# junhong-3dv/s2m2

Measured on AMD Instinct MI355X. Metric: stereo pairs/sec, S-model 1216x1024 fp16 refine_iter=3 (ms/pair = 1000*n_gpus/value), higher is better.
Workload: dtype f16; 1 GPU; S-model 1216x1024 refine_iter=3 use_positivity=True, 1 pair(s) per GPU per step, random-init weights (seeded LeCun normal); pairs_per_gpu=1, parallelism=dp1 (pairs sharded, RCCL gather of outputs to rank 0)

## Files before the change

__graft_entry__.py:

```python
import os
import sys

ROOT = os.path.dirname(os.path.abspath(__file__))
if ROOT not in sys.path:
    sys.path.insert(0, ROOT)


def build() -> None:
    from s2m2_amd.build import build as build_lib
    lib = build_lib(verbose=True)
    assert os.path.exists(lib)
    _check_isa()
    import s2m2_amd
    from s2m2_amd import hip
    hip.load()
    import oracle.s2m2_oracle
    _build_ref()
    print("[build] ok:", lib)


def _build_ref() -> None:
    from oracle import make_ref, ref_loader
    if os.path.isdir(make_ref.SRC):
        make_ref.build(verbose=True)
    print("[build] oracle/_ref:", "ok" if ref_loader.available() else f"absent ({ref_loader.why_not()})")


def _check_isa() -> None:
    from s2m2_amd import build as B
    csrc = os.path.join(ROOT, "s2m2_amd", "csrc")
    if "-DS2M2_UNTRACKED_LOADS=0" in B.effective_defines():
        print("[build] check_isa: skipped (tracked loads: nothing to guard)")
        return
    stamp = os.path.join(B.OBJ, f"check_isa.{B.config_key()}.ok")
    newest = max(os.path.getmtime(os.path.join(csrc, f)) for f in os.listdir(csrc) if f in ("conv.hip", "conv_narrow.hip", "fusion.hip", "ln_corr.hip") or f.endswith(".h"))
    newest = max(newest, os.path.getmtime(os.path.join(ROOT, "tools", "check_isa.py")))
    if os.path.exists(stamp) and os.path.getmtime(stamp) > newest:
        print("[build] check_isa: up to date")
        return
    import subprocess
    r = subprocess.run([sys.executable, os.path.join(ROOT, "tools", "check_isa.py")], capture_output=True, text=True)
    sys.stdout.write(r.stdout)
    if r.returncode != 0:
        if os.environ.get("S2M2_ISA_FALLBACK") == "1":
            print("[build] check_isa failed (assertions above): S2M2_ISA_FALLBACK=1 -> rebuilding with tracked loads (-DS2M2_UNTRACKED_LOADS=0)")
            B.build(force=True, verbose=True, extra_defines=("-DS2M2_UNTRACKED_LOADS=0",))
            return
        raise RuntimeError("tools/check_isa.py failed -- the violated assertions:\n" + r.stdout + r.stderr[-2000:] +
                           "\n(S2M2_ISA_FALLBACK=1 rebuilds the library with tracked loads instead of failing)")
    open(stamp, "w").write("ok\n")


def smoke() -> None:
    import torch
    from oracle import s2m2_oracle as O
    from s2m2_amd.model import S2M2
    from s2m2_amd.weights import seeded_state_dict, synthetic_pair
    assert torch.cuda.is_available(), "smoke() needs cuda:0"
# ... 27 lines not shown
```

include/s2m2_hip.h:

```cpp
#ifndef S2M2_HIP_H
#define S2M2_HIP_H

#include <stddef.h>
#include <stdint.h>

#ifdef __cplusplus
extern "C" {
#endif

enum { S2M2_F32 = 0, S2M2_F16 = 1 };

#define S2M2_ABI_VERSION 800
int s2m2_version(void);
const char* s2m2_last_error(void);
int s2m2_debug_poison_lds(void* stream);
int s2m2_debug_clock_probe(void* out, void* stream);

const char* s2m2_ln_corr_kernel_name(int C, int feat_dtype, int cv_dtype);

typedef struct s2m2_corr_desc {
    const void* tokens;
    const float* ln_weight;
    const float* ln_bias;
    void* cv;
// ... 152 lines not shown
} s2m2_rowattn_desc;
int s2m2_row_attn_supported(int C, int heads, int w, int dtype);
int s2m2_row_attn(const s2m2_rowattn_desc* desc, void* stream);

typedef struct s2m2_convblock_desc {
    const void* x;
    long long x_stride;
    void* out;
    long long out_stride;
    int N, H, W, C;
    const void* w_conv0;
    const void* w_conv2;
    const void* w_1x0;
    const void* w_1x2;
    const float* b_conv0;
    const float* b_conv2;
    const float* b_1x0;
    const float* b_1x2;
    int patch_rows;
    int dtype;
} s2m2_convblock_desc;
int s2m2_conv_block_supported(int C, int H, int W, int dtype);
int s2m2_conv_block(const s2m2_convblock_desc* desc, void* stream);

typedef struct s2m2_pw_desc {
    const void* src[4];
    int src_c[4];
    long long src_stride[4];
    int nsrc;
    long long rows;
    const void* weight_frag;
    const float* bias;
    void* out;
    long long out_stride;
    int Cout;
    int act;
    int shuffle2, Ho, Wo;
    int dtype;
} s2m2_pw_desc;
int s2m2_pw_direct_supported(int K, int Cout, int dtype);
int s2m2_pw_direct(const s2m2_pw_desc* desc, void* stream);

typedef struct s2m2_narrow_desc {
    const void* x;
    long long x_stride;
    int N, H, W, Cin;
// ... 111 lines not shown
```

s2m2_amd/csrc/convblock.hip:

```cpp
#include "common.h"
#include "launch.h"
#include "plan.h"
#include "epilogue.h"
#include <stdlib.h>

namespace s2m2 {

struct CbArgs {
    const half_t* x; half_t* out;
    long long xs, os;
    int N, H, W, tiles_x, tiles_y;
    const raw16_t* w1; const raw16_t* w2;
    const raw16_t* wa; const raw16_t* wb;
    const float* b1; const float* b2; const float* ba; const float* bb;
    const void* zero;
};

template <int C_, int PH_>
struct CbCfg {
    static constexpr int C = C_, PH = PH_, PW = 32, NW = C_ / 32, NT = 64 * NW, KS = 8, CH = 128, NCHUNK = C_ / 128;
    static constexpr int IH = PH + 2, IW = PW + 2, NI = IH * IW, MT1 = (NI + 31) / 32;
    static constexpr int HH = PH + 4, HW = PW + 4, NHALO = HH * HW;
    static constexpr int RS = CH + 8, TRS = C + 8;
    static constexpr int PPX = CH / 8, RPI = NT / PPX, A_IT = (NHALO + RPI - 1) / RPI, AROWS = A_IT * RPI;
    static constexpr size_t A_BYTES = (size_t)AROWS * RS * 2;
    static constexpr size_t R_BYTES = (size_t)PH * 32 * TRS * 2;
    static constexpr size_t T_BYTES = (size_t)MT1 * 32 * TRS * 2;
    static constexpr size_t A_REGION = A_BYTES > R_BYTES ? A_BYTES : R_BYTES;
    static constexpr size_t OFF_T = (A_REGION + 15) / 16 * 16, OFF_B = OFF_T + T_BYTES, LDS_BYTES = OFF_B + 4 * C * 4;
    static_assert(LDS_BYTES <= 160 * 1024 && NT % PPX == 0, "conv block tile");
};

template <int MT, int KS>
__device__ __forceinline__ void cb_steps(float16_t (&acc)[MT], const half_t* a, const int (&poff)[MT], raw16_t (&ring)[KS], const raw16_t* wf,
                                         int& g, int nfrag) {
    Frag<half_t> xf[2][MT];
#pragma unroll
    for (int i = 0; i < MT; ++i) load_frag(xf[0][i], a + poff[i]);
#pragma unroll
    for (int kk = 0; kk < KS; ++kk) {
        if (kk + 1 < KS) {
#pragma unroll
            for (int i = 0; i < MT; ++i) load_frag(xf[(kk + 1) & 1][i], a + poff[i] + (kk + 1) * 16);
        }
        wait_vmcnt<KS - 2>();
        settle(ring[kk]);
        Frag<half_t> wfr;
        wfr.v = __builtin_bit_cast(half8_t, ring[kk]);
#pragma unroll
        for (int i = 0; i < MT; ++i) mma32(acc[i], wfr, xf[kk & 1][i]);
        {
            const int f = g + KS - 1;
            global_load16_async(ring[(kk + KS - 1) % KS], wf + (size_t)(f < nfrag ? f : nfrag - 1) * 64);
        }
        ++g;
    }
}

template <typename CFG>
__global__ __launch_bounds__(CFG::NT) void conv_block_kernel(CbArgs p) {
    constexpr int C = CFG::C, PH = CFG::PH, KS = CFG::KS, RS = CFG::RS, TRS = CFG::TRS, HW = CFG::HW, IW = CFG::IW, MT1 = CFG::MT1, NCHUNK = CFG::NCHUNK;
    extern __shared__ __attribute__((aligned(16))) char smem[];
    half_t* Ah = reinterpret_cast<half_t*>(smem);
    half_t* Rt = reinterpret_cast<half_t*>(smem);
    half_t* Tt = reinterpret_cast<half_t*>(smem + CFG::OFF_T);
    float* bvec = reinterpret_cast<float*>(smem + CFG::OFF_B);
    const int tid = threadIdx.x, lane = tid & 63, l31 = lane & 31, hi = lane >> 5;
    const int wv = __builtin_amdgcn_readfirstlane(tid >> 6);
    int bx = blockIdx.x;
    const int tx = bx % p.tiles_x; bx /= p.tiles_x;
    const int ty = bx % p.tiles_y;
    const int n = bx / p.tiles_y;
    const int y0 = ty * PH, x0 = tx * 32;

    for (int i = tid; i < 4 * C; i += CFG::NT) {
        const int k = i / C, c = i - k * C;
        const float* src = k == 0 ? p.b1 : k == 1 ? p.b2 : k == 2 ? p.ba : p.bb;
        bvec[i] = src ? src[c] : 0.f;
    }
    const int pc = tid % CFG::PPX, prow = tid / CFG::PPX;
// ... 218 lines not shown
```

s2m2_amd/csrc/plan.h:

```cpp
#pragma once
#include <stddef.h>
#include <type_traits>
#include <vector>
#include "common.h"

namespace s2m2 {

bool plan_recording();
constexpr int kPlanMaskWords = 4;
struct PlanPtrMask {
    unsigned long long bits[kPlanMaskWords] = {0, 0, 0, 0};
    bool overflow = false;
    void set(size_t byte_off) {
        const size_t w = byte_off / 8;
        if (byte_off % 8 != 0 || w >= 64 * kPlanMaskWords) overflow = true;
        else bits[w / 64] |= 1ULL << (w % 64);
    }
    bool test(size_t w) const { return w < 64 * kPlanMaskWords && ((bits[w / 64] >> (w % 64)) & 1ULL) != 0; }
};
int plan_append(int (*tramp)(const void* blob, void* stream), const void* blob, size_t bytes, const char* name, const PlanPtrMask& mask);

struct PlanEntry {
    const char* name;
    int (*tramp)(const void* blob, void* stream);
// ... 67 lines not shown
            for (size_t o : offs) m.set(base + o);                                                                  \
        }                                                                                                           \
    };
#define S2M2_OFF(D, f) offsetof(D, f)
#define S2M2_OFF_I(D, f, i) (offsetof(D, f) + 8 * (i))
S2M2_PLAN_PTRS(s2m2_corr_desc, S2M2_OFF(s2m2_corr_desc, tokens), S2M2_OFF(s2m2_corr_desc, ln_weight), S2M2_OFF(s2m2_corr_desc, ln_bias),
               S2M2_OFF(s2m2_corr_desc, cv), S2M2_OFF(s2m2_corr_desc, start_event), S2M2_OFF(s2m2_corr_desc, stop_event))
S2M2_PLAN_PTRS(s2m2_conv_desc, S2M2_OFF_I(s2m2_conv_desc, src, 0), S2M2_OFF_I(s2m2_conv_desc, src, 1), S2M2_OFF_I(s2m2_conv_desc, src, 2),
               S2M2_OFF_I(s2m2_conv_desc, src, 3), S2M2_OFF(s2m2_conv_desc, weight), S2M2_OFF(s2m2_conv_desc, bias), S2M2_OFF(s2m2_conv_desc, out),
               S2M2_OFF(s2m2_conv_desc, aux0), S2M2_OFF(s2m2_conv_desc, aux1), S2M2_OFF(s2m2_conv_desc, ln_wsum), S2M2_OFF(s2m2_conv_desc, bias2))
S2M2_PLAN_PTRS(s2m2_chain_desc, S2M2_OFF(s2m2_chain_desc, x), S2M2_OFF(s2m2_chain_desc, res), S2M2_OFF(s2m2_chain_desc, out),
               S2M2_OFF_I(s2m2_chain_desc, weight, 0), S2M2_OFF_I(s2m2_chain_desc, weight, 1), S2M2_OFF_I(s2m2_chain_desc, weight, 2),
               S2M2_OFF_I(s2m2_chain_desc, bias, 0), S2M2_OFF_I(s2m2_chain_desc, bias, 1), S2M2_OFF_I(s2m2_chain_desc, bias, 2),
               S2M2_OFF_I(s2m2_chain_desc, ln_wsum, 0), S2M2_OFF_I(s2m2_chain_desc, ln_wsum, 1), S2M2_OFF_I(s2m2_chain_desc, ln_wsum, 2),
               S2M2_OFF(s2m2_chain_desc, ln_out), S2M2_OFF(s2m2_chain_desc, ln_gamma), S2M2_OFF(s2m2_chain_desc, ln_beta),
               S2M2_OFF(s2m2_chain_desc, fan_weight), S2M2_OFF(s2m2_chain_desc, fan_bias), S2M2_OFF(s2m2_chain_desc, fan_ln_wsum),
               S2M2_OFF(s2m2_chain_desc, fan_out))
S2M2_PLAN_PTRS(s2m2_rowattn_desc, S2M2_OFF(s2m2_rowattn_desc, x), S2M2_OFF(s2m2_rowattn_desc, out), S2M2_OFF(s2m2_rowattn_desc, weights),
               S2M2_OFF(s2m2_rowattn_desc, vectors), S2M2_OFF(s2m2_rowattn_desc, ln_out))
S2M2_PLAN_PTRS(s2m2_convblock_desc, S2M2_OFF(s2m2_convblock_desc, x), S2M2_OFF(s2m2_convblock_desc, out), S2M2_OFF(s2m2_convblock_desc, w_conv0),
               S2M2_OFF(s2m2_convblock_desc, w_conv2), S2M2_OFF(s2m2_convblock_desc, w_1x0), S2M2_OFF(s2m2_convblock_desc, w_1x2),
               S2M2_OFF(s2m2_convblock_desc, b_conv0), S2M2_OFF(s2m2_convblock_desc, b_conv2), S2M2_OFF(s2m2_convblock_desc, b_1x0),
               S2M2_OFF(s2m2_convblock_desc, b_1x2))
S2M2_PLAN_PTRS(s2m2_pw_desc, S2M2_OFF_I(s2m2_pw_desc, src, 0), S2M2_OFF_I(s2m2_pw_desc, src, 1), S2M2_OFF_I(s2m2_pw_desc, src, 2),
               S2M2_OFF_I(s2m2_pw_desc, src, 3), S2M2_OFF(s2m2_pw_desc, weight_frag), S2M2_OFF(s2m2_pw_desc, bias), S2M2_OFF(s2m2_pw_desc, out))
S2M2_PLAN_PTRS(s2m2_narrow_desc, S2M2_OFF(s2m2_narrow_desc, x), S2M2_OFF(s2m2_narrow_desc, x1), S2M2_OFF(s2m2_narrow_desc, weight_frag),
               S2M2_OFF(s2m2_narrow_desc, bias), S2M2_OFF(s2m2_narrow_desc, out), S2M2_OFF(s2m2_narrow_desc, head_frag),
               S2M2_OFF(s2m2_narrow_desc, head_bias))

template <typename D> struct PlanDescBlob { int (*impl)(const D*, void*); D desc; };
template <typename D> int plan_desc_tramp(const void* blob, void* stream) {
    const auto* b = static_cast<const PlanDescBlob<D>*>(blob);
    return b->impl(&b->desc, stream);
}
template <typename D> int plan_dispatch_desc(const char* name, int (*impl)(const D*, void*), const D* d, void* stream) {
#if S2M2_RANGE_CHECK
    range_bind_tu();
    const int rc = impl(d, stream) || range_collect(name, stream);
#else
    const int rc = impl(d, stream);
#endif
    if (rc == 0 && d && plan_recording()) {
        PlanDescBlob<D> b;
        __builtin_memset(&b, 0, sizeof(b));
        b.impl = impl;
        b.desc = *d;
// ... 31 lines not shown
```

s2m2_amd/engine.py:

```python
from __future__ import annotations

import os
from dataclasses import dataclass
from functools import cached_property
from typing import Dict, Optional, Sequence, Tuple

import torch
import torch.nn.functional as F

from . import hip, pack

Tensor = torch.Tensor


@dataclass(eq=False)
class Layer:
    weight: Tensor
    bias: Optional[Tensor]
    kh: int
    kw: int
    cout: int
    korder: int = 0

    def __post_init__(self):
# ... 81 lines not shown
        self.use_positivity = model.use_positivity
        self.refine_iter = model.refine_iter
        self.output_upsample = model.output_upsample
        self.device = next(model.parameters()).device
        self.p: Dict[str, Tensor] = {n: q.detach().to(self.device, torch.float32) for n, q in model.named_parameters()}
        self._layers: Dict[object, Layer] = {}
        self._composites: Dict[object, object] = {}
        self._supported: Dict[tuple, object] = {}
        self._pe_cache: Dict[Tuple[int, int], Tuple[Tensor, Tensor]] = {}
        self._bufs: Dict[object, Tensor] = {}
        self._plans: Dict[object, object] = {}
        self._ns = None
        self.fuse_k1ln = os.environ.get("S2M2_FUSE_K1LN", "1") != "0"
        self.cv_band = 11 if (os.environ.get("S2M2_CV_BAND", "0") == "1" and self.use_positivity) else -1
        self.use_k12 = os.environ.get("S2M2_K12", "1") != "0"
        self.use_k12_head = self.use_k12 and os.environ.get("S2M2_K12_HEAD", "1") != "0"
        self.native_refine = os.environ.get("S2M2_REFINE_NATIVE", "1") != "0"
        self.use_rowfuse = os.environ.get("S2M2_ROWFUSE", "1") != "0"
        self.coarse_fuse = os.environ.get("S2M2_COARSE_FUSE", "1") != "0"
        self.use_convblock = os.environ.get("S2M2_CONVBLOCK", "1") != "0"
        self.convblock_maxpix = int(os.environ.get("S2M2_CONVBLOCK_MAXPIX", "40000"))
        self.convblock_c256 = os.environ.get("S2M2_CONVBLOCK_C256", "0") == "1"
        self.gru_frag = os.environ.get("S2M2_GRU_FRAG", "0") == "1"
        self._tokens_normed: Optional[Tensor] = None
        self.ln_w = self.p["disp_init.layer_norm.weight"].contiguous()
        self.ln_b = self.p["disp_init.layer_norm.bias"].contiguous()
        self.k1_events = None

    def std(self, name: str, splits: Optional[Sequence[Tuple[int, int]]] = None, transposed: bool = False, frag: bool = True) -> Layer:
        key = (name, tuple(splits) if splits else None, transposed, bool(frag))
        s = self._layers.get(key)
        if s is None:
            w = self.p[name + ".weight"]
            if transposed:
                w = pack.convT_s1_as_conv(w)
            if w.dim() == 2:
                w = w[:, :, None, None]
            cin_p = sum(pd for _, pd in splits) if splits else pack.pad8(w.shape[1])
            frag = frag and pack.frag_eligible(pack.pad8(w.shape[0]), cin_p, w.shape[2], w.shape[3], self.dtype)
            wp = pack.pack_conv_frag(w, self.dtype, splits) if frag else pack.pack_conv(w, self.dtype, splits)
            s = self._layers[key] = Layer(wp, pack.pack_bias(self.p.get(name + ".bias"), w.shape[0]), w.shape[2], w.shape[3],
                                          pack.pad8(w.shape[0]), 2 if frag else 0)
        return s

    def merged(self, key: str, parts: Sequence[Tuple[str, int, float, bool]], cin_total: int) -> Layer:
        s = self._layers.get(key)
# ... 161 lines not shown
            return hip.conv2d([gf], dual[0], dual[1], 1, 1, dual[0].shape[0], act=hip.ACT_SIGMOID, epi=hip.EPI_DUALMIX, aux0=z0, aux1=z1,
                              ksplit=cg, bias2=dual[2])
        m = self.cconv(self.std(p + ".feature_gate.2"), [gf[..., :cg]], act=hip.ACT_SIGMOID, epi=hip.EPI_GATEMIX, aux0=z0, aux1=z1)
        return self.cconv(self.std(p + ".feature_fusion.2"), [gf[..., cg:]], epi=hip.EPI_ADD, aux0=m)

    def chain_ok(self, c: int) -> bool:
        return self.supported("mlp_chain", c)

    def chain_frag_ok(self, c: int) -> bool:
        return self.supported("mlp_chain_frag", c)

    def fusion_frag_ok(self, c: int) -> bool:
        return self.supported("feature_fusion_frag", c)

    def fusion_ok(self, c: int) -> bool:
        return self.supported("feature_fusion", c) or self.fusion_frag_ok(c)

    def pw_ok(self, k: int, cout: int) -> bool:
        return self.supported("pw_direct", k, cout)

    def narrow_ok(self, kh: int, kw: int, stride: int, cin: int, cout: int) -> bool:
        return self.use_k12 and self.supported("conv_narrow", kh, kw, stride, cin, cout)

    def convblock_ok(self, c: int, h: int, w: int) -> bool:
        return self.supported("conv_block", c, h, w)

    def row_ok(self, z: Tensor, nh: int) -> bool:
        return self.use_rowfuse and z.dim() == 4 and self.supported("row_attn", z.shape[-1], nh, z.shape[2])

    def pe(self, h: int, w: int) -> Tuple[Tensor, Tensor]:
        key = (h, w)
        if key not in self._pe_cache:
            self._pe_cache[key] = pe_tables(h, w, self.device)
        return self._pe_cache[key]

    def qkv_spec(self, p: str) -> Layer:
        c = self.p[p + ".q.weight"].shape[1]
        return self.merged(p + "|qkv", [(p + ".q", 0, 1.0, False), (p + ".k", 0, 1.0, False), (p + ".v", 0, 1.0, False)], c)

    def qkv(self, p: str, x: Tensor) -> Tensor:
        spec = self.qkv_spec(p)
        c = x.shape[-1]
        if spec.is_1x1 and spec.cout == 3 * c and self.chain_frag_ok(c):
            return hip.mlp_fan(x, *spec.fan())
        return self.cconv(spec, [x], ln=True)

# ... 115 lines not shown
        tail = self.up_tail(p + ".up_concat2", z2.shape[-1], p + ".up_conv2", z3.shape[-1])
        up3 = None
        for k, bp in enumerate(blocks):
            last = k + 1 == len(blocks)
            z3, q = self.attn_block(bp, z3, 8, True, qkv_in=q, next_block=None if last else blocks[k + 1], tail=tail if last else None)
            if last and tail is not None:
                up3, q = q, None
        z2 = self.attn_block(p + ".dec_attn2", self.fusion_up(p + ".up_concat2", z2, p + ".up_conv2", z3, up_pre=up3), 4, False)[0]
        z1 = self.attn_block(p + ".dec_attn1", self.fusion_up(p + ".up_concat1", z1, p + ".up_conv1", z2), 2, False)[0]
        z0 = self.attn_block(p + ".dec_attn0", self.fusion_up(p + ".up_concat0", z0, p + ".up_conv0", z1), 1, False, ln_out=ln_out)[0]
        return z0, z1, z2, z3

    def global_refiner(self, p: str, ctx: Tensor, disp: Tensor, conf: Tensor) -> Tensor:
        small = hip.refine_prep(disp, conf, None, 0, self.dtype)
        f = self.cconv(self.std(p + ".init_feat.0", splits=[(2, 8), (self.C, self.C)]), [small, ctx], act=hip.ACT_GELU)
        f = self.cconv(self.std(p + ".init_feat.2"), [f])
        f = self.unet(p + ".refine_unet", f)[0]
        return hip.global_update(self.cconv(self.std(p + ".out_feat.0"), [f]), disp, conf, self.use_positivity)

    def gru(self, p: str, h: Tensor, x: Tensor) -> Tensor:
        C = h.shape[-1]
        for sfx in ("1", "2"):
            zr = self.merged(f"{p}|zr{sfx}", [(f"{p}.convz{sfx}", 0, 1.0, False), (f"{p}.convr{sfx}", 0, 1.0, False)], h.shape[-1] + x.shape[-1])
            if zr.korder == 2 and zr.cout == 2 * C and C % 128 == 0:
                both = self.cconv(zr, [h, x], act=hip.ACT_SIGMOID, epi=hip.EPI_MUL, aux0=h, epi_cout0=C)
                z, rh = both[..., :C], both[..., C:]
            else:
                z = self.cconv(self.std(f"{p}.convz{sfx}"), [h, x], act=hip.ACT_SIGMOID)
                rh = self.cconv(self.std(f"{p}.convr{sfx}"), [h, x], act=hip.ACT_SIGMOID, epi=hip.EPI_MUL, aux0=h)
            h = self.cconv(self.std(f"{p}.convq{sfx}", frag=self.gru_frag), [rh, x], act=hip.ACT_TANH, epi=hip.EPI_GRU, aux0=z, aux1=h)
        return h

    def local_refiner(self, p: str, hidden: Tensor, ctx: Tensor, disp: Tensor, conf: Tensor, occ: Tensor, cv: Tensor, cap, it,
                      small: Optional[Tensor] = None, want_small: bool = False):
        B, _, h, w = disp.shape
        C = self.C
        sa = self.merged(p + "|corrA", [(p + ".corr_feat1.0", 0, 1 / 16, False), (p + ".corr_feat2.0", 16, 1 / 16, False)], 32)
        sb = self.merged(p + "|corrB", [(p + ".corr_feat1.2", 0, 1.0, False), (p + ".corr_feat2.2", 96, 1.0, False)], 192)
        corr = self.zeros("lr_corr", (B, h, w, 32))
        hip.cv_lookup_into(cv, disp.contiguous(), corr, 0, 16, 4)
        f12 = self.cconv(sb, [self.cconv(sa, [corr], act=hip.ACT_GELU)])
        if cap is not None:
            cap[f"corr1_it{it}"], cap[f"corr2_it{it}"] = (corr[..., 0:9].permute(0, 3, 1, 2).clone(),
                                                          corr[..., 16:25].permute(0, 3, 1, 2).clone())
        if small is None:
            small = hip.refine_prep(disp, conf, occ, 1, self.dtype)
# ... 282 lines not shown
```

s2m2_amd/hip.py:

```python
from __future__ import annotations

import contextlib
import ctypes
import os
from typing import Optional, Tuple

import torch

_HERE = os.path.dirname(os.path.abspath(__file__))
LIB_PATH = os.path.join(_HERE, "lib", "libs2m2_hip%s.so" % os.environ.get("S2M2_LIB_SUFFIX", ""))

F32, F16 = 0, 1
_DT = {torch.float32: F32, torch.float16: F16}

_lib: Optional[ctypes.CDLL] = None

_vp, _i, _ll = ctypes.c_void_p, ctypes.c_int, ctypes.c_longlong

ACT_NONE, ACT_GELU, ACT_RELU, ACT_SIGMOID, ACT_TANH = 0, 1, 2, 3, 4
EPI_NONE, EPI_ADD, EPI_MUL, EPI_GRU, EPI_GATEMIX, EPI_DUALMIX = 0, 1, 2, 3, 4, 5


class ConvDesc(ctypes.Structure):
    _fields_ = [("src", _vp * 4), ("src_c", _i * 4), ("src_stride", _i * 4), ("nsrc", _i), ("weight", _vp), ("bias", _vp),
# ... 2 lines not shown
                ("out_scale", ctypes.c_float), ("shuffle2", _i), ("tile", _i), ("dtype", _i), ("korder", _i), ("stride", _i),
                ("ln_wsum", _vp), ("ln_eps", ctypes.c_float), ("ksplit", _i), ("bias2", _vp), ("pool2", _i), ("epi_cout0", _i)]


class ChainDesc(ctypes.Structure):
    _fields_ = [("x", _vp), ("res", _vp), ("out", _vp), ("x_stride", _ll), ("res_stride", _ll), ("out_stride", _ll), ("rows", _ll),
                ("C", _i), ("nstage", _i), ("weight", _vp * 3), ("bias", _vp * 3), ("ln_wsum", _vp * 3), ("act", _i * 3),
                ("res_stage", _i), ("carry", _i), ("ln_eps", ctypes.c_float), ("dtype", _i),
                ("ln_out", _vp), ("ln_out_stride", _ll), ("ln_gamma", _vp), ("ln_beta", _vp), ("ln_out_eps", ctypes.c_float),
                ("fan_weight", _vp), ("fan_bias", _vp), ("fan_ln_wsum", _vp), ("fan_out", _vp), ("fan_out_stride", _ll),
                ("nfan", _i), ("xcd_group_rows", _ll), ("weight_frag", _i), ("pool_h", _i), ("pool_w", _i)]


class RowAttnDesc(ctypes.Structure):
    _fields_ = [("x", _vp), ("x_stride", _ll), ("out", _vp), ("out_stride", _ll), ("nimg", _i), ("h", _i), ("w", _i), ("C", _i), ("heads", _i),
                ("cross", _i), ("weights", _vp), ("vectors", _vp), ("ln_eps", ctypes.c_float),
                ("ln_out", _vp), ("ln_out_stride", _ll), ("ln_out_eps", ctypes.c_float), ("xcd_hint", _i), ("dtype", _i)]


class ConvBlockDesc(ctypes.Structure):
    _fields_ = [("x", _vp), ("x_stride", _ll), ("out", _vp), ("out_stride", _ll), ("N", _i), ("H", _i), ("W", _i), ("C", _i),
                ("w_conv0", _vp), ("w_conv2", _vp), ("w_1x0", _vp), ("w_1x2", _vp), ("b_conv0", _vp), ("b_conv2", _vp), ("b_1x0", _vp),
                ("b_1x2", _vp), ("patch_rows", _i), ("dtype", _i)]


class PwDesc(ctypes.Structure):
    _fields_ = [("src", _vp * 4), ("src_c", _i * 4), ("src_stride", _ll * 4), ("nsrc", _i), ("rows", _ll), ("weight_frag", _vp), ("bias", _vp),
                ("out", _vp), ("out_stride", _ll), ("Cout", _i), ("act", _i), ("shuffle2", _i), ("Ho", _i), ("Wo", _i), ("dtype", _i)]


class NarrowDesc(ctypes.Structure):
    _fields_ = [("x", _vp), ("x_stride", _ll), ("N", _i), ("H", _i), ("W", _i), ("Cin", _i), ("x1", _vp), ("x1_stride", _ll), ("Cin1", _i),
                ("weight_frag", _vp), ("bias", _vp), ("out", _vp), ("out_stride", _ll), ("Cout", _i), ("KH", _i), ("KW", _i), ("stride", _i),
                ("act", _i), ("dtype", _i), ("head_frag", _vp), ("head_bias", _vp), ("head_cout", _i)]


class CorrDesc(ctypes.Structure):
    _fields_ = [("tokens", _vp), ("ln_weight", _vp), ("ln_bias", _vp), ("cv", _vp), ("B", _i), ("h", _i), ("w", _i), ("C", _i),
                ("cv_pitch", _i), ("band", _i), ("token_dtype", _i), ("cv_dtype", _i), ("start_event", _vp), ("stop_event", _vp)]


class PackDesc(ctypes.Structure):
    _fields_ = [("kind", _i), ("w", _vp), ("w2", _vp), ("rows", _i), ("cols", _i), ("ld", _i), ("ld2", _i), ("ntap", _i), ("out", _vp),
                ("out_elems", _ll)]


# ... 48 lines not shown
    "s2m2_engine_load": (_i, [ctypes.c_char_p, ctypes.POINTER(_vp)]),
    "s2m2_engine_meta": (_i, [_vp, ctypes.POINTER(EngineInfo)]),
    "s2m2_engine_run": (_i, [_vp, _vp, _vp, _vp, _vp, _vp, _vp]),
    "s2m2_engine_destroy": (_i, [_vp]),
    "s2m2_pack_frag_elems": (_ll, [ctypes.POINTER(PackDesc)]),
    "s2m2_pack_frag": (_i, [ctypes.POINTER(PackDesc), _vp]),
    "s2m2_event_create": (_i, [ctypes.POINTER(_vp)]),
    "s2m2_event_destroy": (_i, [_vp]),
    "s2m2_event_elapsed_us": (_i, [_vp, _vp, ctypes.POINTER(ctypes.c_float)]),
    "s2m2_sinkhorn_workspace_bytes": (ctypes.c_size_t, [_i, _i, _i, _i]),
    "s2m2_pw_direct_supported": (_i, [_i, _i, _i]),
    "s2m2_pw_direct": (_i, [ctypes.POINTER(PwDesc), _vp]),
    "s2m2_conv_narrow_supported": (_i, [_i, _i, _i, _i, _i, _i]),
    "s2m2_conv_narrow": (_i, [ctypes.POINTER(NarrowDesc), _vp]),
    "s2m2_sinkhorn_regress": (_i, [_vp, _vp, _vp, _vp, _vp, _i, _i, _i, _i, _i, _i, _i, _vp, _vp]),
    "s2m2_cv_lookup": (_i, [_vp, _vp, _vp, _vp, _i, _i, _i, _i, _i, _i, _ll, _ll, _ll, _i, _vp]),
    "s2m2_conv2d": (_i, [ctypes.POINTER(ConvDesc), _vp]),
    "s2m2_mlp_chain_supported": (_i, [_i, _i]),
    "s2m2_mlp_chain_frag_supported": (_i, [_i, _i]),
    "s2m2_mlp_fan_supported": (_i, [_i, _i, _i]),
    "s2m2_mlp_chain": (_i, [ctypes.POINTER(ChainDesc), _vp]),
    "s2m2_conv_block_supported": (_i, [_i, _i, _i, _i]),
    "s2m2_conv_block": (_i, [ctypes.POINTER(ConvBlockDesc), _vp]),
    "s2m2_row_attn_supported": (_i, [_i, _i, _i, _i]),
    "s2m2_row_attn": (_i, [ctypes.POINTER(RowAttnDesc), _vp]),
    "s2m2_feature_fusion_supported": (_i, [_i, _i]),
    "s2m2_feature_fusion": (_i, [_vp, _vp, _vp, _ll, _ll, _ll, _ll, _i, _vp, _vp, _vp, _vp, _vp, _i, _i, _i, _vp]),
    "s2m2_feature_fusion_frag_supported": (_i, [_i, _i]),
    "s2m2_feature_fusion_frag": (_i, [_vp, _vp, _vp, _ll, _ll, _ll, _ll, _i, _vp, _vp, _vp, _vp, _i, _i, _i, _vp]),
    "s2m2_convex_upsample": (_i, [_vp, _vp, _vp, _i, _vp, _i, _i, _i, _i, _i, _i, _vp, _ll, _i, _vp]),
    "s2m2_attention": (_i, [_vp, _vp, _vp, _vp, _ll, _ll, _ll, _ll, _i, _i, _i, _i, _i, ctypes.c_float, _i, _vp, _vp, _vp, _ll,
                            _i, _i, _i, _vp]),
    "s2m2_attention_supported": (_i, [_i, _i, _i, _i, _i, _i, _i]),
    "s2m2_resample2x": (_i, [_vp, _vp, _i, _i, _i, _i, _ll, _ll, _i, _i, _vp]),
    "s2m2_image_prep": (_i, [_vp, _vp, _vp, _i, _i, _i, _i, _i, _vp]),
    "s2m2_refine_prep": (_i, [_vp, _vp, _vp, _vp, _ll, _i, _i, _vp]),
    "s2m2_global_update": (_i, [_vp, _i, _vp, _vp, _vp, _ll, _i, _i, _vp]),
    "s2m2_refine_update": (_i, [_vp, _i, _vp, _vp, _vp, _ll, _i, _i, _i, _vp]),
    "s2m2_debug_poison_lds": (_i, [_vp]),
    "s2m2_debug_clock_probe": (_i, [_vp, _vp]),
    "s2m2_refine_update_to": (_i, [_vp, _i, _vp, _vp, _vp, _vp, _vp, _vp, _vp, _ll, _i, _i, _i, _vp]),
    "s2m2_tanh": (_i, [_vp, _vp, _ll, _i, _vp]),
    "s2m2_stem_mlp": (_i, [_vp, _vp, _vp, _vp, _vp, _vp, _ll, _i, _vp]),
    "s2m2_image_pad": (_i, [_vp, _vp, _vp, _i, _i, _i, _i, _i, _i, _vp]),
    "s2m2_layernorm": (_i, [_vp, _vp, _ll, _i, _ll, _ll, _i, _vp]),
    "s2m2_groupnorm_workspace_bytes": (ctypes.c_size_t, [_i, _i]),
# ... 892 lines not shown
    if records.dtype != torch.float32 or records.dim() != 2 or records.shape[1] != RECTIFY_RECORD_FLOATS or records.shape[0] < 1:
        raise ValueError(f"rectify: records must be an (n_img, {RECTIFY_RECORD_FLOATS}) fp32 tensor")
    n = records.shape[0]
    if out is None and maps is None:
        raise ValueError("rectify: no output requested")
    ref = out if out is not None else maps
    if ref.dim() != 4:
        raise ValueError("rectify: out is (n_img,3,Hd,Wd), maps is (n_img,2,Hd,Wd)")
    Hd, Wd = (hd, wd) if hd is not None and wd is not None else ref.shape[-2:]
    d = RectifyDesc()
    if out is not None:
        if out.dtype not in (torch.float32, torch.uint8):
            raise ValueError("rectify: out must be an (n_img,3,Hd,Wd) fp32 or uint8 tensor")
        _mat(out, (n, 3, Hd, Wd), out.dtype, "rectify: out")
        d.out, d.out_dtype = out.data_ptr(), _IMG_DT[out.dtype]
        d.src[0], d.src[1] = srcs[0].data_ptr(), srcs[-1].data_ptr()
    if maps is not None:
        _mat(maps, (n, 2, Hd, Wd), torch.float32, "rectify: maps")
        d.maps = maps.data_ptr()
    d.records, d.n_src, d.n_img, d.Hs, d.Ws, d.Hd, d.Wd = records.data_ptr(), len(srcs), n, Hs, Ws, Hd, Wd
    d.src_format, d.round, d.order = fmt, int(bool(round)), order
    with torch.cuda.device(records.device):
        _check(load().s2m2_rectify(ctypes.byref(d), _stream()), "s2m2_rectify")
```

Measured before the change: 127.4 pairs/s.

## Fuse separable ConvGRU half-step into one kernel computing z, r, q and update

Adds a conv_gru HIP kernel that loads an h/x tile with halo into LDS, computes the z and r gates on separate wave groups, scales the r-gated h in LDS, runs the q convolution and applies the GRU combine in a single launch, for the 1x3 and 3x1 ConvGRU steps at C=128. It replaces the previous path of a merged zr conv with epilogue followed by a separate q conv and combine, which avoids intermediate global round trips and extra launches. The shared MFMA weight ring helper moves into a header. The cost is recomputing halo rows for r (and half the waves sit idle during the q stage), plus added LDS pressure. The path is on by default through S2M2_GRU_FUSE.

```diff
diff --git a/__graft_entry__.py b/__graft_entry__.py
--- a/__graft_entry__.py
+++ b/__graft_entry__.py
@@ -33,7 +33,7 @@
         print("[build] check_isa: skipped (tracked loads: nothing to guard)")
         return
     stamp = os.path.join(B.OBJ, f"check_isa.{B.config_key()}.ok")
-    newest = max(os.path.getmtime(os.path.join(csrc, f)) for f in os.listdir(csrc) if f in ("conv.hip", "conv_narrow.hip", "fusion.hip", "ln_corr.hip") or f.endswith(".h"))
+    newest = max(os.path.getmtime(os.path.join(csrc, f)) for f in os.listdir(csrc) if f in ("conv.hip", "conv_narrow.hip", "fusion.hip", "ln_corr.hip", "convblock.hip", "convgru.hip") or f.endswith(".h"))
     newest = max(newest, os.path.getmtime(os.path.join(ROOT, "tools", "check_isa.py")))
     if os.path.exists(stamp) and os.path.getmtime(stamp) > newest:
         print("[build] check_isa: up to date")
diff --git a/include/s2m2_hip.h b/include/s2m2_hip.h
--- a/include/s2m2_hip.h
+++ b/include/s2m2_hip.h
@@ -198,6 +198,24 @@
 } s2m2_convblock_desc;
 int s2m2_conv_block_supported(int C, int H, int W, int dtype);
 int s2m2_conv_block(const s2m2_convblock_desc* desc, void* stream);
+
+typedef struct s2m2_convgru_desc {
+    const void* h;
+    long long h_stride;
+    const void* x;
+    long long x_stride;
+    void* out;
+    long long out_stride;
+    int N, H, W, C;
+    int KH, KW;
+    const void* w_zr;
+    const void* w_q;
+    const float* b_zr;
+    const float* b_q;
+    int dtype;
+} s2m2_convgru_desc;
+int s2m2_conv_gru_supported(int C, int H, int W, int dtype);
+int s2m2_conv_gru(const s2m2_convgru_desc* desc, void* stream);
 
 typedef struct s2m2_pw_desc {
     const void* src[4];
diff --git a/s2m2_amd/csrc/convblock.hip b/s2m2_amd/csrc/convblock.hip
--- a/s2m2_amd/csrc/convblock.hip
+++ b/s2m2_amd/csrc/convblock.hip
@@ -2,6 +2,7 @@
 #include "launch.h"
 #include "plan.h"
 #include "epilogue.h"
+#include "frag_ring.h"
 #include <stdlib.h>
 
 namespace s2m2 {
@@ -30,32 +31,6 @@
     static constexpr size_t OFF_T = (A_REGION + 15) / 16 * 16, OFF_B = OFF_T + T_BYTES, LDS_BYTES = OFF_B + 4 * C * 4;
     static_assert(LDS_BYTES <= 160 * 1024 && NT % PPX == 0, "conv block tile");
 };
-
-template <int MT, int KS>
-__device__ __forceinline__ void cb_steps(float16_t (&acc)[MT], const half_t* a, const int (&poff)[MT], raw16_t (&ring)[KS], const raw16_t* wf,
-                                         int& g, int nfrag) {
-    Frag<half_t> xf[2][MT];
-#pragma unroll
-    for (int i = 0; i < MT; ++i) load_frag(xf[0][i], a + poff[i]);
-#pragma unroll
-    for (int kk = 0; kk < KS; ++kk) {
-        if (kk + 1 < KS) {
-#pragma unroll
-            for (int i = 0; i < MT; ++i) load_frag(xf[(kk + 1) & 1][i], a + poff[i] + (kk + 1) * 16);
-        }
-        wait_vmcnt<KS - 2>();
-        settle(ring[kk]);
-        Frag<half_t> wfr;
-        wfr.v = __builtin_bit_cast(half8_t, ring[kk]);
-#pragma unroll
-        for (int i = 0; i < MT; ++i) mma32(acc[i], wfr, xf[kk & 1][i]);
-        {
-            const int f = g + KS - 1;
-            global_load16_async(ring[(kk + KS - 1) % KS], wf + (size_t)(f < nfrag ? f : nfrag - 1) * 64);
-        }
-        ++g;
-    }
-}
 
 template <typename CFG>
 __global__ __launch_bounds__(CFG::NT) void conv_block_kernel(CbArgs p) {
diff --git a/s2m2_amd/csrc/convgru.hip b/s2m2_amd/csrc/convgru.hip
--- /dev/null
+++ b/s2m2_amd/csrc/convgru.hip
@@ -0,0 +1,243 @@
+#include "common.h"
+#include "launch.h"
+#include "plan.h"
+#include "epilogue.h"
+#include "frag_ring.h"
+#include <stdint.h>
+
+namespace s2m2 {
+
+struct GruArgs {
+    const half_t* h; const half_t* x; half_t* out;
+    long long hs, xs, os;
+    int N, H, W, tiles_x, tiles_y;
+    const raw16_t* wzr; const raw16_t* wq;
+    const float* bzr; const float* bq;
+    const void* zero;
+};
+
+template <bool VERT_>
+struct GruCfg {
+    static constexpr bool VERT = VERT_;
+    static constexpr int C = 128, KS = 8, NWAVES = 8, NT = 64 * NWAVES, NTAP = 3, NFRAG = 2 * NTAP * KS;
+    static constexpr int PH = VERT ? 8 : 4, PW = VERT ? 20 : 40, NP = PH * PW, MTZ = NP / 32;
+    static constexpr int RH = VERT ? PH + 2 : PH, RW = VERT ? PW : PW + 2, NR = RH * RW, MTR = (NR + 31) / 32;
+    static constexpr int TH = VERT ? PH + 4 : PH, TW = VERT ? PW : PW + 4, NTILE = TH * TW;
+    static constexpr int TAPS = VERT ? TW : 1;
+    static constexpr int RS = C + 8, CRS = C + 8;
+    static constexpr int PPX = C / 8, RPI = NT / PPX, A_IT = (NTILE + RPI - 1) / RPI, AROWS = A_IT * RPI;
+    static constexpr size_t A_BYTES = (size_t)AROWS * RS * 2;
+    static constexpr size_t STAGE_BYTES = (size_t)NP * CRS * 2;
+    static constexpr size_t OFF_X = A_BYTES, OFF_B = 2 * A_BYTES, LDS_BYTES = OFF_B + 3 * C * 4;
+    static constexpr int PCR = C / 8, SP = NP * PCR / NT;
+    static_assert(NP % 32 == 0 && NP * PCR % NT == 0 && STAGE_BYTES <= A_BYTES && LDS_BYTES <= 160 * 1024, "conv gru tile");
+};
+
+template <typename CFG, int MT>
+__device__ __forceinline__ void gru_layer(float16_t (&acc)[MT], const half_t* t0, const half_t* t1, const int (&poff)[MT], const raw16_t* wf) {
+    constexpr int KS = CFG::KS;
+    raw16_t ring[KS];
+#pragma unroll
+    for (int i = 0; i < MT; ++i)
+#pragma unroll
+        for (int r = 0; r < 16; ++r) acc[i][r] = 0.f;
+#pragma unroll
+    for (int s = 0; s < KS - 1; ++s) global_load16_async(ring[s], wf + (size_t)s * 64);
+    int g = 0;
+#pragma unroll 1
+    for (int chunk = 0; chunk < 2; ++chunk) {
+        const half_t* t = chunk ? t1 : t0;
+#pragma unroll 1
+        for (int tap = 0; tap < CFG::NTAP; ++tap) cb_steps<MT, KS>(acc, t + tap * CFG::TAPS * CFG::RS, poff, ring, wf, g, CFG::NFRAG);
+    }
+    wait_vmcnt<0>();
+#pragma unroll
+    for (int s = 0; s < KS; ++s) settle(ring[s]);
+}
+
+template <int ACT>
+__device__ __forceinline__ void gate16(half4_t (&o)[4], const float16_t& acc, const float* bv, int hi) {
+#pragma unroll
+    for (int gq = 0; gq < 4; ++gq) {
+        const float4_t b = *reinterpret_cast<const float4_t*>(bv + 8 * gq + 4 * hi);
+#pragma unroll
+        for (int e = 0; e < 4; ++e) {
+            float v = activate<ACT>(acc[4 * gq + e] + b[e]);
+            asm volatile("" : "+v"(v));
+            o[gq][e] = from_f32<half_t>(v);
+        }
+    }
+}
+
+template <typename CFG>
+__global__ __launch_bounds__(CFG::NT) void conv_gru_kernel(GruArgs p) {
+    constexpr int RS = CFG::RS, CRS = CFG::CRS, TW = CFG::TW, PW = CFG::PW, RW = CFG::RW, MTZ = CFG::MTZ, MTR = CFG::MTR, C = CFG::C;
+    extern __shared__ __attribute__((aligned(16))) char smem[];
+    half_t* Ht = reinterpret_cast<half_t*>(smem);
+    half_t* Xt = reinterpret_cast<half_t*>(smem + CFG::OFF_X);
+    half_t* Zs = Ht;
+    half_t* Qs = Xt;
+    float* bvec = reinterpret_cast<float*>(smem + CFG::OFF_B);
+    const int tid = threadIdx.x, lane = tid & 63, l31 = lane & 31, hi = lane >> 5;
+    const int wv = __builtin_amdgcn_readfirstlane(tid >> 6);
+    int bx = blockIdx.x;
+    const int tx = bx % p.tiles_x; bx /= p.tiles_x;
+    const int ty = bx % p.tiles_y;
+    const int n = bx / p.tiles_y;
+    const int y0 = ty * CFG::PH, x0 = tx * PW;
+    const half_t* zp = static_cast<const half_t*>(p.zero);
+
+    for (int i = tid; i < 3 * C; i += CFG::NT) {
+        const float* src = i < 2 * C ? p.bzr : p.bq;
+        bvec[i] = src ? src[i < 2 * C ? i : i - 2 * C] : 0.f;
+    }
+    {
+        const int pc = tid % CFG::PPX, prow = tid / CFG::PPX;
+        long long apix[CFG::A_IT];
+#pragma unroll
+        for (int it = 0; it < CFG::A_IT; ++it) {
+            const int tp = prow + CFG::RPI * it;
+            const int tyy = tp / TW, txx = tp - tyy * TW;
+            const int yy = y0 + tyy - (CFG::VERT ? 2 : 0), xx = x0 + txx - (CFG::VERT ? 0 : 2);
+            const bool ok = tp < CFG::NTILE && yy >= 0 && yy < p.H && xx >= 0 && xx < p.W;
+            apix[it] = ok ? ((long long)(n * p.H + yy) * p.W + xx) : -1;
+        }
+        raw16_t ra[CFG::A_IT];
+#pragma unroll
+        for (int it = 0; it < CFG::A_IT; ++it) ra[it] = global_load16(apix[it] >= 0 ? p.h + apix[it] * p.hs + pc * 8 : zp);
+#pragma unroll
+        for (int it = 0; it < CFG::A_IT; ++it) *reinterpret_cast<raw16_t*>(Ht + (size_t)(prow + CFG::RPI * it) * RS + pc * 8) = ra[it];
+#pragma unroll
+        for (int it = 0; it < CFG::A_IT; ++it) ra[it] = global_load16(apix[it] >= 0 ? p.x + apix[it] * p.xs + pc * 8 : zp);
+#pragma unroll
+        for (int it = 0; it < CFG::A_IT; ++it) *reinterpret_cast<raw16_t*>(Xt + (size_t)(prow + CFG::RPI * it) * RS + pc * 8) = ra[it];
+    }
+    __syncthreads();
+
+    int poffZ[MTZ], poffR[MTR];
+#pragma unroll
+    for (int i = 0; i < MTZ; ++i) {
+        const int q = 32 * i + l31, py = q / PW, px = q - py * PW;
+        poffZ[i] = ((CFG::VERT ? (py + 1) * TW + px : py * TW + px + 1)) * RS + hi * 8;
+    }
+#pragma unroll
+    for (int i = 0; i < MTR; ++i) {
+        int q = 32 * i + l31;
+        q = q < CFG::NR ? q : CFG::NR - 1;
+        const int ry = q / RW, rx = q - ry * RW;
+        poffR[i] = (ry * TW + rx) * RS + hi * 8;
+    }
+
+    const raw16_t* wf1 = p.wzr + (size_t)wv * CFG::NFRAG * 64 + lane;
+    half4_t gate[MTR][4];
+    if (wv < 4) {
+        float16_t acc[MTZ];
+        gru_layer<CFG, MTZ>(acc, Ht, Xt, poffZ, wf1);
+#pragma unroll
+        for (int i = 0; i < MTZ; ++i) gate16<S2M2_ACT_SIGMOID>(gate[i], acc[i], bvec + wv * 32, hi);
+    } else {
+        float16_t acc[MTR];
+        gru_layer<CFG, MTR>(acc, Ht, Xt, poffR, wf1);
+#pragma unroll
+        for (int i = 0; i < MTR; ++i) gate16<S2M2_ACT_SIGMOID>(gate[i], acc[i], bvec + wv * 32, hi);
+    }
+    __syncthreads();
+    if (wv >= 4) {
+#pragma unroll
+        for (int i = 0; i < MTR; ++i) {
+            if (32 * i + l31 < CFG::NR) {
+                half_t* row = Ht + (poffR[i] - hi * 8) + CFG::TAPS * RS + (wv - 4) * 32 + 4 * hi;
+#pragma unroll
+                for (int gq = 0; gq < 4; ++gq) {
+                    half4_t hv = *reinterpret_cast<const half4_t*>(row + 8 * gq);
+#pragma unroll
+                    for (int e = 0; e < 4; ++e) hv[e] = from_f32<half_t>(to_f32(gate[i][gq][e]) * to_f32(hv[e]));
+                    *reinterpret_cast<half4_t*>(row + 8 * gq) = hv;
+                }
+            }
+        }
+    }
+    __syncthreads();
+
+    half4_t cand[MTZ][4];
+    if (wv < 4) {
+        float16_t acc[MTZ];
+        gru_layer<CFG, MTZ>(acc, Ht, Xt, poffZ, p.wq + (size_t)wv * CFG::NFRAG * 64 + lane);
+#pragma unroll
+        for (int i = 0; i < MTZ; ++i) gate16<S2M2_ACT_TANH>(cand[i], acc[i], bvec + 2 * C + wv * 32, hi);
+    }
+    __syncthreads();
+
+    raw16_t hreg[CFG::SP];
+    long long opix[CFG::SP];
+#pragma unroll
+    for (int it = 0; it < CFG::SP; ++it) {
+        const int s = tid + CFG::NT * it, r = s / CFG::PCR, pcc = s - r * CFG::PCR;
+        const int py = r / PW, yy = y0 + py, xx = x0 + (r - py * PW);
+        opix[it] = (yy < p.H && xx < p.W) ? ((long long)(n * p.H + yy) * p.W + xx) : -1;
+        hreg[it] = global_load16(opix[it] >= 0 ? p.h + opix[it] * p.hs + pcc * 8 : zp);
+    }
+    if (wv < 4) {
+#pragma unroll
+        for (int i = 0; i < MTZ; ++i) {
+            const size_t o = (size_t)(32 * i + l31) * CRS + wv * 32 + 4 * hi;
+#pragma unroll
+            for (int gq = 0; gq < 4; ++gq) {
+                *reinterpret_cast<half4_t*>(Zs + o + 8 * gq) = gate[i][gq];
+                *reinterpret_cast<half4_t*>(Qs + o + 8 * gq) = cand[i][gq];
+            }
+        }
+    }
+    __syncthreads();
+#pragma unroll
+    for (int it = 0; it < CFG::SP; ++it) {
+        const int s = tid + CFG::NT * it, r = s / CFG::PCR, pcc = s - r * CFG::PCR;
+        if (opix[it] < 0) continue;
+        Vec16<half_t> v = *reinterpret_cast<const Vec16<half_t>*>(Qs + (size_t)r * CRS + pcc * 8);
+        const Vec16<half_t> zv = *reinterpret_cast<const Vec16<half_t>*>(Zs + (size_t)r * CRS + pcc * 8);
+        aux_combine(v, (int)S2M2_EPI_GRU, zv, __builtin_bit_cast(Vec16<half_t>, hreg[it]));
+        *reinterpret_cast<Vec16<half_t>*>(p.out + opix[it] * p.os + pcc * 8) = v;
+    }
+}
+
+template <bool VERT>
+static int launch_gru(const GruArgs& a0, hipStream_t st) {
+    using CFG = GruCfg<VERT>;
+    GruArgs a = a0;
+    a.tiles_x = (a.W + CFG::PW - 1) / CFG::PW;
+    a.tiles_y = (a.H + CFG::PH - 1) / CFG::PH;
+    return launch<conv_gru_kernel<CFG>>("conv_gru", dim3((unsigned)(a.N * a.tiles_x * a.tiles_y)), dim3(CFG::NT), CFG::LDS_BYTES, st, a);
+}
+
+}
+
+extern "C" int s2m2_conv_gru_supported(int C, int H, int W, int dtype) {
+    return dtype == S2M2_F16 && C == 128 && H >= 1 && W >= 1;
+}
+
+static int conv_gru_impl(const s2m2_convgru_desc* d, void* stream) {
+    using namespace s2m2;
+    S2M2_REQUIRE(d, "conv_gru: null descriptor");
+    S2M2_REQUIRE(d->dtype == S2M2_F16 && d->C == 128, "conv_gru: C=%d dtype=%d (fp16, C = 128)", d->C, d->dtype);
+    S2M2_REQUIRE((d->KH == 3 && d->KW == 1) || (d->KH == 1 && d->KW == 3), "conv_gru: %d x %d taps (3 x 1 or 1 x 3)", d->KH, d->KW);
+    S2M2_REQUIRE(d->h && d->x && d->out && d->out != d->h && d->out != d->x, "conv_gru: h / x / out must be non-null, out distinct from both");
+    S2M2_REQUIRE(d->N > 0 && d->H > 0 && d->W > 0 && (long long)d->N * d->H * d->W < (1LL << 24), "conv_gru: bad shape");
+    S2M2_REQUIRE(d->h_stride >= d->C && d->h_stride % 8 == 0 && d->x_stride >= d->C && d->x_stride % 8 == 0 && d->out_stride >= d->C &&
+                 d->out_stride % 8 == 0, "conv_gru: pixel strides (at least C, multiples of 8)");
+    S2M2_REQUIRE(((uintptr_t)d->h | (uintptr_t)d->x | (uintptr_t)d->out) % 16 == 0, "conv_gru: h / x / out must be 16-byte aligned");
+    S2M2_REQUIRE(d->w_zr && d->w_q, "conv_gru: null weight");
+    GruArgs a;
+    a.h = static_cast<const half_t*>(d->h); a.x = static_cast<const half_t*>(d->x); a.out = static_cast<half_t*>(d->out);
+    a.hs = d->h_stride; a.xs = d->x_stride; a.os = d->out_stride;
+    a.N = d->N; a.H = d->H; a.W = d->W;
+    a.wzr = static_cast<const raw16_t*>(d->w_zr); a.wq = static_cast<const raw16_t*>(d->w_q);
+    a.bzr = d->b_zr; a.bq = d->b_q;
+    if (bind_zero_page(a, "conv_gru")) return 1;
+    hipStream_t st = static_cast<hipStream_t>(stream);
+    return d->KH == 3 ? launch_gru<true>(a, st) : launch_gru<false>(a, st);
+}
+static constexpr char kConvGruEntry[] = "s2m2_conv_gru";
+extern "C" int s2m2_conv_gru(const s2m2_convgru_desc* d, void* stream) {
+    return s2m2::plan_dispatch_desc<s2m2_convgru_desc>(kConvGruEntry, &conv_gru_impl, d, stream);
+}
+S2M2_PLAN_DESC_ENTRY(kConvGruEntry, conv_gru_impl)
diff --git a/s2m2_amd/csrc/frag_ring.h b/s2m2_amd/csrc/frag_ring.h
--- /dev/null
+++ b/s2m2_amd/csrc/frag_ring.h
@@ -0,0 +1,32 @@
+#pragma once
+#include "common.h"
+
+namespace s2m2 {
+
+template <int MT, int KS>
+__device__ __forceinline__ void cb_steps(float16_t (&acc)[MT], const half_t* a, const int (&poff)[MT], raw16_t (&ring)[KS], const raw16_t* wf,
+                                         int& g, int nfrag) {
+    Frag<half_t> xf[2][MT];
+#pragma unroll
+    for (int i = 0; i < MT; ++i) load_frag(xf[0][i], a + poff[i]);
+#pragma unroll
+    for (int kk = 0; kk < KS; ++kk) {
+        if (kk + 1 < KS) {
+#pragma unroll
+            for (int i = 0; i < MT; ++i) load_frag(xf[(kk + 1) & 1][i], a + poff[i] + (kk + 1) * 16);
+        }
+        wait_vmcnt<KS - 2>();
+        settle(ring[kk]);
+        Frag<half_t> wfr;
+        wfr.v = __builtin_bit_cast(half8_t, ring[kk]);
+#pragma unroll
+        for (int i = 0; i < MT; ++i) mma32(acc[i], wfr, xf[kk & 1][i]);
+        {
+            const int f = g + KS - 1;
+            global_load16_async(ring[(kk + KS - 1) % KS], wf + (size_t)(f < nfrag ? f : nfrag - 1) * 64);
+        }
+        ++g;
+    }
+}
+
+}
diff --git a/s2m2_amd/csrc/plan.h b/s2m2_amd/csrc/plan.h
--- a/s2m2_amd/csrc/plan.h
+++ b/s2m2_amd/csrc/plan.h
@@ -113,6 +113,9 @@
                S2M2_OFF(s2m2_convblock_desc, w_conv2), S2M2_OFF(s2m2_convblock_desc, w_1x0), S2M2_OFF(s2m2_convblock_desc, w_1x2),
                S2M2_OFF(s2m2_convblock_desc, b_conv0), S2M2_OFF(s2m2_convblock_desc, b_conv2), S2M2_OFF(s2m2_convblock_desc, b_1x0),
                S2M2_OFF(s2m2_convblock_desc, b_1x2))
+S2M2_PLAN_PTRS(s2m2_convgru_desc, S2M2_OFF(s2m2_convgru_desc, h), S2M2_OFF(s2m2_convgru_desc, x), S2M2_OFF(s2m2_convgru_desc, out),
+               S2M2_OFF(s2m2_convgru_desc, w_zr), S2M2_OFF(s2m2_convgru_desc, w_q), S2M2_OFF(s2m2_convgru_desc, b_zr),
+               S2M2_OFF(s2m2_convgru_desc, b_q))
 S2M2_PLAN_PTRS(s2m2_pw_desc, S2M2_OFF_I(s2m2_pw_desc, src, 0), S2M2_OFF_I(s2m2_pw_desc, src, 1), S2M2_OFF_I(s2m2_pw_desc, src, 2),
                S2M2_OFF_I(s2m2_pw_desc, src, 3), S2M2_OFF(s2m2_pw_desc, weight_frag), S2M2_OFF(s2m2_pw_desc, bias), S2M2_OFF(s2m2_pw_desc, out))
 S2M2_PLAN_PTRS(s2m2_narrow_desc, S2M2_OFF(s2m2_narrow_desc, x), S2M2_OFF(s2m2_narrow_desc, x1), S2M2_OFF(s2m2_narrow_desc, weight_frag),
diff --git a/s2m2_amd/engine.py b/s2m2_amd/engine.py
--- a/s2m2_amd/engine.py
+++ b/s2m2_amd/engine.py
@@ -127,6 +127,7 @@
         self.convblock_maxpix = int(os.environ.get("S2M2_CONVBLOCK_MAXPIX", "40000"))
         self.convblock_c256 = os.environ.get("S2M2_CONVBLOCK_C256", "0") == "1"
         self.gru_frag = os.environ.get("S2M2_GRU_FRAG", "0") == "1"
+        self.gru_fuse = os.environ.get("S2M2_GRU_FUSE", "1") != "0"
         self._tokens_normed: Optional[Tensor] = None
         self.ln_w = self.p["disp_init.layer_norm.weight"].contiguous()
         self.ln_b = self.p["disp_init.layer_norm.bias"].contiguous()
@@ -334,6 +335,9 @@
     def narrow_ok(self, kh: int, kw: int, stride: int, cin: int, cout: int) -> bool:
         return self.use_k12 and self.supported("conv_narrow", kh, kw, stride, cin, cout)
 
+    def gru_fuse_ok(self, c: int, h: int, w: int) -> bool:
+        return getattr(hip, "conv_gru_supported", None) is not None and self.supported("conv_gru", c, h, w)
+
     def convblock_ok(self, c: int, h: int, w: int) -> bool:
         return self.supported("conv_block", c, h, w)
 
@@ -495,6 +499,11 @@
         C = h.shape[-1]
         for sfx in ("1", "2"):
             zr = self.merged(f"{p}|zr{sfx}", [(f"{p}.convz{sfx}", 0, 1.0, False), (f"{p}.convr{sfx}", 0, 1.0, False)], h.shape[-1] + x.shape[-1])
+            if self.gru_fuse and zr.korder == 2 and zr.cout == 2 * C and x.shape[-1] == C and h.dim() == 4 and self.gru_fuse_ok(C, h.shape[1], h.shape[2]):
+                q = self.std(f"{p}.convq{sfx}")
+                if q.korder == 2 and q.cout == C and (q.kh, q.kw) == (zr.kh, zr.kw) and (q.kh, q.kw) in ((1, 3), (3, 1)):
+                    h = hip.conv_gru(h, x, zr.weight, zr.bias, q.weight, q.bias, q.kh, q.kw)
+                    continue
             if zr.korder == 2 and zr.cout == 2 * C and C % 128 == 0:
                 both = self.cconv(zr, [h, x], act=hip.ACT_SIGMOID, epi=hip.EPI_MUL, aux0=h, epi_cout0=C)
                 z, rh = both[..., :C], both[..., C:]
diff --git a/s2m2_amd/hip.py b/s2m2_amd/hip.py
--- a/s2m2_amd/hip.py
+++ b/s2m2_amd/hip.py
@@ -48,6 +48,11 @@
     _fields_ = [("x", _vp), ("x_stride", _ll), ("out", _vp), ("out_stride", _ll), ("N", _i), ("H", _i), ("W", _i), ("C", _i),
                 ("w_conv0", _vp), ("w_conv2", _vp), ("w_1x0", _vp), ("w_1x2", _vp), ("b_conv0", _vp), ("b_conv2", _vp), ("b_1x0", _vp),
                 ("b_1x2", _vp), ("patch_rows", _i), ("dtype", _i)]
+
+
+class ConvGruDesc(ctypes.Structure):
+    _fields_ = [("h", _vp), ("h_stride", _ll), ("x", _vp), ("x_stride", _ll), ("out", _vp), ("out_stride", _ll), ("N", _i), ("H", _i), ("W", _i),
+                ("C", _i), ("KH", _i), ("KW", _i), ("w_zr", _vp), ("w_q", _vp), ("b_zr", _vp), ("b_q", _vp), ("dtype", _i)]
 
 
 class PwDesc(ctypes.Structure):
@@ -142,6 +147,8 @@
     "s2m2_mlp_chain": (_i, [ctypes.POINTER(ChainDesc), _vp]),
     "s2m2_conv_block_supported": (_i, [_i, _i, _i, _i]),
     "s2m2_conv_block": (_i, [ctypes.POINTER(ConvBlockDesc), _vp]),
+    "s2m2_conv_gru_supported": (_i, [_i, _i, _i, _i]),
+    "s2m2_conv_gru": (_i, [ctypes.POINTER(ConvGruDesc), _vp]),
     "s2m2_row_attn_supported": (_i, [_i, _i, _i, _i]),
     "s2m2_row_attn": (_i, [ctypes.POINTER(RowAttnDesc), _vp]),
     "s2m2_feature_fusion_supported": (_i, [_i, _i]),
@@ -1080,3 +1087,6 @@
     d.src_format, d.round, d.order = fmt, int(bool(round)), order
     with torch.cuda.device(records.device):
         _check(load().s2m2_rectify(ctypes.byref(d), _stream()), "s2m2_rectify")
+
+
+from .hip_gru import conv_gru, conv_gru_supported
diff --git a/s2m2_amd/hip_gru.py b/s2m2_amd/hip_gru.py
--- /dev/null
+++ b/s2m2_amd/hip_gru.py
@@ -0,0 +1,29 @@
+import ctypes
+
+import torch
+
+from . import hip as _h
+
+
+def conv_gru_supported(C: int, H: int, W: int, dtype: torch.dtype) -> bool:
+    return bool(_h.load().s2m2_conv_gru_supported(C, H, W, _h._DT[dtype]))
+
+
+def conv_gru(h: torch.Tensor, x: torch.Tensor, w_zr: torch.Tensor, b_zr, w_q: torch.Tensor, b_q, KH: int, KW: int) -> torch.Tensor:
+    _h._resident("conv_gru", h, x, w_zr, b_zr, w_q, b_q)
+    if h.dtype != torch.float16 or x.dtype != torch.float16 or tuple(h.shape) != tuple(x.shape):
+        raise ValueError("conv_gru: h and x must be (N,H,W,C) fp16 tensors of one shape")
+    hs, xs = _h._pixels(h, "conv_gru: h"), _h._pixels(x, "conv_gru: x")
+    N, H, W, C = h.shape
+    _h._vec(w_zr, 2 * C * KH * KW * 2 * C, "conv_gru: w_zr", dtype=h.dtype)
+    _h._vec(w_q, C * KH * KW * 2 * C, "conv_gru: w_q", dtype=h.dtype)
+    _h._vec(b_zr, 2 * C, "conv_gru: b_zr", optional=True)
+    _h._vec(b_q, C, "conv_gru: b_q", optional=True)
+    d = _h.ConvGruDesc()
+    out = torch.empty((N, H, W, C), device=h.device, dtype=h.dtype)
+    d.h, d.h_stride, d.x, d.x_stride, d.out, d.out_stride = h.data_ptr(), hs, x.data_ptr(), xs, out.data_ptr(), C
+    d.N, d.H, d.W, d.C, d.KH, d.KW = N, H, W, C, KH, KW
+    d.w_zr, d.w_q, d.b_zr, d.b_q, d.dtype = w_zr.data_ptr(), w_q.data_ptr(), _h._ptr(b_zr), _h._ptr(b_q), _h._DT[h.dtype]
+    _h._check(_h.load().s2m2_conv_gru(ctypes.byref(d), _h._stream()), "s2m2_conv_gru")
+    _h._meter("conv_gru", 2.0 * N * H * W * (3 * C) * (2 * C) * KH * KW)
+    return out
```

New measurement: 131.5 pairs/s, median of 6. 3.3% higher.
